# Hjinhan/Transgo

Measured on AMD Instinct MI355X. Metric: MCTS simulations/sec, higher is better.
Workload: dtype f32

## Files before the change

transgo_amd/csrc/net.hip:

```cpp
#include <cmath>
#include <cstdlib>
#include <cstring>
#include <string>
#include <vector>

#include "conv_rows.h"
#include "engine.h"

using namespace tg;

namespace tg {

struct ConvW { const float* w; const float* b; };
struct BlockW { const float* s1; const float* t1; ConvW c1; ConvW c2; const float* g1; const float* g2;
                const _Float16* h1; const _Float16* h2; };
struct AttW { ConvW qkv; const float* gamma; const float* s; const float* t;
              const _Float16* x3w = nullptr; const float* x3sc = nullptr; };
struct Layer { int kind; int ridx; AttW a; };

enum Chain { CHAIN_F32 = 0, CHAIN_DMA, CHAIN_F16, CHAIN_SPLIT };
struct NetPath {
    Chain chain = CHAIN_F32;
    bool r16 = false;
    bool att_x3 = false;
// ... 209 lines not shown
                if (m >= 0 && m < M) xreg[i] = *reinterpret_cast<const f32x4*>(in + (size_t)m * CIN + cc + c4 * 4);
            }
        }
    };
    auto store_x = [&](int cc) {
#pragma unroll
        for (int i = 0; i < XL; ++i) {
            const int idx = tid + i * 256;
            if (idx < NROW * C4) {
                const int r = idx / C4, c4 = idx % C4;
                f32x4 v = xreg[i];
                if (PRO) {
                    const int m = m0 - HALO + r;
                    if (m >= 0 && m < M) {
                        const f32x4 sc = *reinterpret_cast<const f32x4*>(ps + cc + c4 * 4);
                        const f32x4 sh = *reinterpret_cast<const f32x4*>(pt + cc + c4 * 4);
#pragma unroll
                        for (int e = 0; e < 4; ++e) { float u = v[e] * sc[e] + sh[e]; v[e] = u > 0.f ? u : 0.f; }
                    }
                }
                *reinterpret_cast<f32x4*>(&xs[r * RS + c4 * 4]) = v;
            }
        }
    };
    load_x(0);
    load_w(0, 0);
    for (int cc = 0; cc < CIN; cc += CC) {
        for (int tap = 0; tap < NTAP; ++tap) {
            if (!WALL || tap == 0) {
                __syncthreads();
                if (tap == 0) store_x(cc);
                store_w();
                __syncthreads();
                if (!WALL && tap < NTAP - 1) load_w(cc, tap + 1);
                else if (cc + CC < CIN) { load_w(cc + CC, 0); load_x(cc + CC); }
            }
            const int toff = NTAP == 9 ? (tap / 3 - 1) * S + (tap % 3 - 1) : 0;
#pragma unroll
            for (int sub = 0; sub < CC / 16; ++sub) {
                f32x4 b[NPT];
#pragma unroll
                for (int t = 0; t < NPT; ++t) {
                    const int r = (wave * NPT + t) * 16 + j + HALO + toff;
                    b[t] = *reinterpret_cast<const f32x4*>(&xs[r * RS + sub * 16 + kq * 4]);
                    if (!((vmask[t] >> tap) & 1)) b[t] = f32x4{0.f, 0.f, 0.f, 0.f};
                }
#pragma unroll
                for (int ct = 0; ct < CT; ++ct) {
                    const f32x4 a = *reinterpret_cast<const f32x4*>(&ws[((WALL ? tap * COUT : 0) + ct * 16 + j) * RS + sub * 16 + kq * 4]);
#pragma unroll
                    for (int s = 0; s < 4; ++s)
#pragma unroll
                        for (int t = 0; t < NPT; ++t)
                            acc[ct][t] = __builtin_amdgcn_mfma_f32_16x16x4f32(a[s], b[t][s], acc[ct][t], 0, 0, 0);
                }
            }
        }
    }
    int mrow[NPT], srow[NPT];
#pragma unroll
    for (int t = 0; t < NPT; ++t) {
        mrow[t] = m0 + (wave * NPT + t) * 16 + j;
        srow[t] = SM2 || SM1 ? conv_sg_row(mrow[t] / P, mrow[t] % P, P) : mrow[t];
    }
    conv_epilogue<COUT, CT, NPT, EPI, SM1, SM2>(acc, mrow, M, 0, kq, out, res, out2, par, srow, conv_sg_rows(M / P, P));
}

typedef __attribute__((address_space(3))) void tg_lds_void;
#define TG_VMCNT(N) asm volatile("s_waitcnt vmcnt(%0)" ::"n"(N) : "memory")
#define TG_BARRIER() do { asm volatile("" ::: "memory"); __builtin_amdgcn_s_barrier(); asm volatile("" ::: "memory"); } while (0)

using u32x4 = __attribute__((ext_vector_type(4))) unsigned int;
__device__ __forceinline__ u32x4 tg_rsrc(const void* base, unsigned bytes) {
    const unsigned long long a = (unsigned long long)base;
    return u32x4{(unsigned)a, (unsigned)(a >> 32) & 0xffffu, bytes, 0x00020000u};
}
__device__ __forceinline__ void tg_dma_global(const void* sbase , int voff_bytes, tg_lds_void* lds) {
    const unsigned la = __builtin_amdgcn_readfirstlane((unsigned)(unsigned long long)lds);
    asm volatile("s_mov_b32 m0, %0\n\ts_nop 0\n\tglobal_load_lds_dwordx4 %1, %2" ::"s"(la), "v"(voff_bytes), "s"(sbase) : "memory");
}
__device__ __forceinline__ void tg_dma_buffer(u32x4 rsrc, int voff_bytes, tg_lds_void* lds) {
    const unsigned la = __builtin_amdgcn_readfirstlane((unsigned)(unsigned long long)lds);
    asm volatile("s_mov_b32 m0, %0\n\ts_nop 0\n\tbuffer_load_dwordx4 %1, %2, 0 offen lds" ::"s"(la), "v"(voff_bytes), "s"(rsrc) : "memory");
}

__device__ __forceinline__ int swz64(int row) { return ((row >> 2) & 1) << 1; }

#ifdef TG_CONV_STAMP
__device__ unsigned long long g_conv_stamp[2 * 6 * 8];
#define TG_CSTAMP(i) do { __builtin_amdgcn_sched_barrier(0); if (cslot >= 0 && lane == 0) g_conv_stamp[cslot * 8 + (i)] = __builtin_readcyclecounter(); \
                          __builtin_amdgcn_sched_barrier(0); } while (0)
#else
#define TG_CSTAMP(i) do { } while (0)
#endif
template <int S, int F, int EPI, bool SIN = false, bool SOUT = false>
__global__ __launch_bounds__(256, (F == 128 ? 4 : 2)) void k_conv3x3_sg(const float* __restrict__ in, float* __restrict__ out,
                                                                       const float* __restrict__ res, const float* __restrict__ Ws,
                                                                       const float* __restrict__ bias, float* __restrict__ out2,
                                                                       const float* __restrict__ s2, const float* __restrict__ t2, int rows) {
    constexpr int P = S * S, CT = F / 16, CC = 16;
    constexpr int NPT = 2, TB = 64 * NPT;
    constexpr int WPW = CT / 4;
    constexpr int NSL = F / CC, D = 4;
    static_assert((F == 128 || F == 256) && NSL % 2 == 0, "tile geometry");
    __shared__ __attribute__((aligned(16))) float ws[D][F * CC];
    __shared__ __attribute__((aligned(16))) float par[3 * F];
    const int tid = threadIdx.x, lane = tid & 63;
    const int wave = __builtin_amdgcn_readfirstlane(tid >> 6);
    const int j = lane & 15, kq = lane >> 4;
#ifdef TG_CONV_STAMP
    const unsigned long long t_entry = __builtin_readcyclecounter();
    __builtin_amdgcn_sched_barrier(0);
#endif
    const int tpx = ((int)gridDim.x + 7) >> 3;
    const int bid = ((int)blockIdx.x & 7) * tpx + ((int)blockIdx.x >> 3);
    const int nrange = (rows + TB - 1) / TB;
    if (bid >= nrange * P) return;
    const int range = bid / P;
    const int p = conv_pos_of(bid - range * P, S);
    const int M = rows * P, Msm = conv_sg_rows(rows, P);
    constexpr bool ACT = EPI == 0 && SIN;
#ifdef TG_CONV_STAMP
    int cslot = -1;
    if (S == 9 && F == 128 && (EPI == 0 || SOUT) && wave == 0 && (range == 0 || range == 7)) {
        const int li = bid - range * P, I = S - 2;
        const int cls = li == 0 ? 0 : li == I * I ? 1 : li == I * I + 4 * I ? 2 : -1;
        if (cls >= 0) cslot = (EPI == 1 ? 6 : 0) + (range == 0 ? 0 : 3) + cls;
    }
    if (cslot >= 0 && lane == 0) g_conv_stamp[cslot * 8] = t_entry;
#endif
    static_assert(F <= 256, "one parameter triple per thread");
    const bool bn = out2 || ACT;
    float pbias = bias[tid & (F - 1)], ps2 = (bn ? s2 : bias)[tid & (F - 1)], pt2 = (bn ? t2 : bias)[tid & (F - 1)];
    __builtin_amdgcn_sched_barrier(0);
    TG_CSTAMP(1);

    const unsigned mask = conv_tap_mask(p, S);
    const int nt = conv_tap_count(mask), nst = NSL * nt;
    const unsigned long long taps = conv_tap_list(mask);
    const int inv = nt == 9 ? 7282 : nt == 6 ? 10923 : 16384;
    auto stage = [&](int k, int* sl, int* tap) {
        *sl = (k * inv) >> 16;
        *tap = (int)(taps >> (4 * (k - *sl * nt))) & 15;
    };

    const __amdgpu_buffer_rsrc_t rin = __builtin_amdgcn_make_buffer_rsrc(const_cast<float*>(in), 0, Msm * F * 4, 0x00020000);
    const int prow = lane >> 2, pchunk = (lane & 3) ^ swz64(lane >> 2);
    auto dma_w = [&](int k) {
        int sl, tap;
        stage(k, &sl, &tap);
        const float* src = Ws + (size_t)(sl * 9 + tap) * (F * CC);
#pragma unroll
        for (int i = 0; i < WPW; ++i) {
            const int pc = wave * WPW + i;
            tg_dma_global(src + pc * 16 * CC, (prow * CC + pchunk * 4) * 4, (tg_lds_void*)(&ws[k & (D - 1)][pc * 256]));
        }
    };
    const int aoff = j * CC + ((kq ^ swz64(j)) << 2);
    const int grp0 = (range * 4 + wave) * NPT;
    const bool active = grp0 * 16 < rows;
    const int boff = ((conv_sg_row(grp0 * 16 + j, p, P)) * CC + kq * 4) * 4;
    f32x4 acc[CT][NPT], b_cur[NPT], b_next[NPT];
    int sl_b = 0, sl_p = -1;
    f32x4 bsc, bsh;
    auto load_b = [&](f32x4* b, int k) {
        int sl, tap;
        stage(k, &sl, &tap);
        sl_b = sl;
        const int ty = (tap * 11) >> 5;
        const int soff = (sl * Msm + ((ty - 1) * S + (tap - 3 * ty - 1)) * 16) * (CC * 4);
#pragma unroll
        for (int t = 0; t < NPT; ++t)
            b[t] = __builtin_bit_cast(f32x4, __builtin_amdgcn_raw_buffer_load_b128(rin, (int)((unsigned)boff + (unsigned)soff + (unsigned)(t * (P * 16 * CC * 4))), 0, 0));
    };
    auto act_b = [&](f32x4* dst, const f32x4* b) {
        if (sl_b != sl_p) {
            sl_p = sl_b;
            bsc = *reinterpret_cast<const f32x4*>(par + F + sl_b * CC + kq * 4);
            bsh = *reinterpret_cast<const f32x4*>(par + 2 * F + sl_b * CC + kq * 4);
        }
#pragma unroll
        for (int t = 0; t < NPT; ++t)
#pragma unroll
            for (int e = 0; e < 4; ++e) dst[t][e] = bn_relu_unpacked(b[t][e], bsc[e], bsh[e]);
    };
    constexpr int NRES = EPI == 1 ? CT * NPT : 0;
#define TG_PAR_LANDED(PATH) asm volatile("; bias, s2, t2 landed: " PATH : "+v"(pbias), "+v"(ps2), "+v"(pt2))
    dma_w(0); dma_w(1);
    TG_CSTAMP(2);
    if (active) {
        load_b(b_cur, 0);
        __builtin_amdgcn_sched_barrier(0);
#pragma unroll
        for (int i = 0; i < CT * NPT; ++i) {
            const int ct = i / NPT, t = i % NPT;
            const int b = (grp0 + t) * 16 + j;
            [[maybe_unused]] const int m = b < rows ? b * P + p : M - 1;
            {
                acc[ct][t] = f32x4{0.f, 0.f, 0.f, 0.f};
                if constexpr (EPI == 1 && SIN) {
                    const __amdgpu_buffer_rsrc_t rres = __builtin_amdgcn_make_buffer_rsrc(const_cast<float*>(res), 0, Msm * F * 4, 0x00020000);
                    acc[ct][t] = __builtin_bit_cast(f32x4, __builtin_amdgcn_raw_buffer_load_b128(rres, (int)((unsigned)boff + (unsigned)(ct * Msm * (CC * 4)) + (unsigned)(t * (P * 16 * CC * 4))), 0, 0));
                } else if constexpr (EPI == 1) {
                    acc[ct][t] = *reinterpret_cast<const f32x4*>(res + (size_t)m * F + ct * 16 + kq * 4);
                }
            }
        }
        TG_VMCNT(NRES + NPT);
        TG_PAR_LANDED("wave with boards");
    } else {
        TG_VMCNT(0);
        TG_PAR_LANDED("wave without boards");
    }
#undef TG_PAR_LANDED
    if (tid < F) { par[tid] = pbias; par[F + tid] = bn ? ps2 : 0.f; par[2 * F + tid] = bn ? pt2 : 0.f; }
    asm volatile("s_waitcnt lgkmcnt(0)" ::: "memory");
    TG_BARRIER();
    TG_CSTAMP(3);
    if constexpr (ACT) {
        if (active) act_b(b_cur, b_cur);
        else {
#pragma unroll
            for (int t = 0; t < NPT; ++t) b_cur[t] = f32x4{0.f, 0.f, 0.f, 0.f};
        }
    }
    if (active) {
#pragma unroll
        for (int t = 0; t < NPT; ++t) {
            if constexpr (!ACT) asm volatile("" : "+v"(b_cur[t]));
            if constexpr (EPI == 1) {
#pragma unroll
                for (int ct = 0; ct < CT; ++ct) asm volatile("" : "+v"(acc[ct][t]));
            }
        }
    }
    dma_w(2); dma_w(3);

    auto walk_stage = [&](int k) {
        const float* wcur = ws[k & (D - 1)];
        load_b(b_next, k + 1);
        __builtin_amdgcn_sched_barrier(0);
        f32x4 a_cur = *reinterpret_cast<const f32x4*>(wcur + aoff);
#pragma unroll
        for (int ct = 0; ct < CT; ++ct) {
            f32x4 a_next = a_cur;
            if (ct + 1 < CT) a_next = *reinterpret_cast<const f32x4*>(wcur + (ct + 1) * 256 + aoff);
#pragma unroll
            for (int s4 = 0; s4 < 4; ++s4)
#pragma unroll
                for (int t = 0; t < NPT; ++t)
                    acc[ct][t] = __builtin_amdgcn_mfma_f32_16x16x4f32(a_cur[s4], b_cur[t][s4], acc[ct][t], 0, 0, 0);
            a_cur = a_next;
#ifdef TG_CONV_STAMP
            if (ct == 0 && k == 0) TG_CSTAMP(4);
#endif
        }
        if constexpr (ACT) {
            __builtin_amdgcn_sched_barrier(0);
            act_b(b_cur, b_next);
        } else {
            __builtin_amdgcn_sched_barrier(0);
#pragma unroll
            for (int t = 0; t < NPT; ++t) {
                asm volatile("" : "+v"(b_next[t]));
                b_cur[t] = b_next[t];
            }
        }
    };
#pragma unroll 1
    for (int k0 = 0; k0 < nst - 2; k0 += 2) {
#pragma unroll
        for (int h = 0; h < 2; ++h) {
            if (active) walk_stage(k0 + h);
            TG_VMCNT(0);
        }
        TG_BARRIER();
        if (k0 + 4 < nst) { dma_w(k0 + 4); dma_w(k0 + 5); }
    }
    if (!active) return;
    walk_stage(nst - 2);
    TG_VMCNT(0);
    constexpr bool SM = EPI == 0 || SOUT;
    const __amdgpu_buffer_rsrc_t rout = __builtin_amdgcn_make_buffer_rsrc(out, 0, (SM ? Msm : M) * F * 4, 0x00020000);
    const unsigned ostep = SM ? (unsigned)Msm * (CC * 4) : CC * 4;
    unsigned ooff[NPT];
#pragma unroll
    for (int t = 0; t < NPT; ++t) {
        const int b = (grp0 + t) * 16 + j;
        ooff[t] = b >= rows ? 0x80000000u : SM ? (unsigned)(conv_sg_row(b, p, P) * CC + kq * 4) * 4 : (unsigned)((b * P + p) * F + kq * 4) * 4;
    }
    auto store_tile = [&](int ct, f32x4 bv) {
#pragma unroll
        for (int t = 0; t < NPT; ++t) {
            f32x4 v = acc[ct][t] + bv;
            if constexpr (EPI == 0) {
#pragma unroll
                for (int e = 0; e < 4; ++e) v[e] = v[e] > 0.f ? v[e] : 0.f;
            }
            __builtin_amdgcn_raw_buffer_store_b128(__builtin_bit_cast(u32x4, v), rout, (int)(ooff[t] + (unsigned)ct * ostep), 0, 0);
        }
    };
    {
        const float* wcur = ws[(nst - 1) & (D - 1)];
        const float* pb = par + kq * 4;
        __builtin_amdgcn_sched_barrier(0);
        f32x4 a_cur = *reinterpret_cast<const f32x4*>(wcur + aoff);
#pragma unroll
        for (int ct = 0; ct < CT; ++ct) {
            f32x4 a_next = a_cur, bv = a_cur;
            if (ct + 1 < CT) a_next = *reinterpret_cast<const f32x4*>(wcur + (ct + 1) * 256 + aoff);
            if (ct > 0) bv = *reinterpret_cast<const f32x4*>(pb + (ct - 1) * 16);
#pragma unroll
            for (int s4 = 0; s4 < 4; ++s4) {
#pragma unroll
                for (int t = 0; t < NPT; ++t)
                    acc[ct][t] = __builtin_amdgcn_mfma_f32_16x16x4f32(a_cur[s4], b_cur[t][s4], acc[ct][t], 0, 0, 0);
                if (s4 == 0 && ct > 0) {
                    __builtin_amdgcn_sched_barrier(0);
                    store_tile(ct - 1, bv);
                    __builtin_amdgcn_sched_barrier(0);
                }
            }
            a_cur = a_next;
        }
        TG_CSTAMP(5);
        __builtin_amdgcn_sched_barrier(0);
        store_tile(CT - 1, *reinterpret_cast<const f32x4*>(pb + (CT - 1) * 16));
    }
#ifdef TG_CONV_STAMP
    TG_CSTAMP(6);
    TG_VMCNT(0);
    TG_CSTAMP(7);
#endif
}

__device__ __forceinline__ size_t h16_index(int m, int c, int M) { return (((size_t)(c >> 5) * 4 + ((c >> 3) & 3)) * M + m) * 8 + (c & 7); }

template <int N>
__device__ __forceinline__ void vmcnt_uniform(int n) {
    if (n >= N) TG_VMCNT(N);
    else if constexpr (N > 0) vmcnt_uniform<N - 1>(n);
}

__device__ __forceinline__ int x2_index(int c) { return ((c >> 4) << 5) + (c & 15); }
template <int F, int CT, int NPT, int EPI, bool R16, bool X2 = false>
__device__ __forceinline__ void conv_epilogue_h8(f32x4 (&acc)[CT][NPT], const int (&mrow)[NPT], int M, int co_base, int kq,
                                                 float* __restrict__ out32, _Float16* __restrict__ out16, const float* par, int pstride,
                                                 float wsc, float& amax) {
    static_assert(CT % 2 == 0, "tile pairs");
    static_assert(!(X2 && R16), "split precision keeps the f32 residual stream");
#pragma unroll
    for (int t = 0; t < NPT; ++t) {
        if (mrow[t] >= M) continue;
#pragma unroll
        for (int u = 0; u < CT / 2; ++u) {
            const int lc = u * 32 + kq * 8, col = co_base + lc;
            f32x4 v[2];
#pragma unroll
            for (int h = 0; h < 2; ++h) v[h] = (X2 ? acc[2 * u + h][t] * wsc : acc[2 * u + h][t]) + *reinterpret_cast<const f32x4*>(par + lc + 4 * h);
            h8 o;
            if constexpr (X2) {
                auto store_split = [&](const f32x4 (&w)[2]) {
                    h8 hi, lo;
#pragma unroll
                    for (int e = 0; e < 8; ++e) { const float x = w[e >> 2][e & 3]; hi[e] = (_Float16)x; lo[e] = (_Float16)(x - (float)hi[e]); }
#pragma unroll
                    for (int e = 0; e < 8; e += 2) amax = __builtin_fmaxf(amax, __builtin_fmaxf(__builtin_fabsf(w[e >> 2][e & 3]), __builtin_fabsf(w[e >> 2][(e & 3) + 1])));
                    const int c2 = x2_index(col);
                    *reinterpret_cast<h8*>(out16 + h16_index(mrow[t], c2, M)) = hi;
                    *reinterpret_cast<h8*>(out16 + h16_index(mrow[t], c2 + 16, M)) = lo;
                };
                if (EPI == 0 || EPI == 4) {
#pragma unroll
                    for (int h = 0; h < 2; ++h)
#pragma unroll
                        for (int e = 0; e < 4; ++e) v[h][e] = v[h][e] > 0.f ? v[h][e] : 0.f;
                }
                if (EPI == 0) { store_split(v); continue; }
                if (out32) {
#pragma unroll
                    for (int h = 0; h < 2; ++h) *reinterpret_cast<f32x4*>(out32 + (size_t)mrow[t] * F + col + 4 * h) = v[h];
                }
                if (out16) {
                    f32x4 w[2];
#pragma unroll
                    for (int h = 0; h < 2; ++h) {
                        const f32x4 sc = *reinterpret_cast<const f32x4*>(par + pstride + lc + 4 * h);
                        const f32x4 sh = *reinterpret_cast<const f32x4*>(par + 2 * pstride + lc + 4 * h);
#pragma unroll
                        for (int e = 0; e < 4; ++e) { const float y = v[h][e] * sc[e] + sh[e]; w[h][e] = y > 0.f ? y : 0.f; }
                    }
                    store_split(w);
                }
                continue;
            }
            if (EPI == 0) {
#pragma unroll
                for (int e = 0; e < 8; ++e) { const float w = v[e >> 2][e & 3]; o[e] = (_Float16)(w > 0.f ? w : 0.f); amax = __builtin_fmaxf(amax, w); }
                *reinterpret_cast<h8*>(out16 + h16_index(mrow[t], col, M)) = o;
            } else {
                if (EPI == 4) {
#pragma unroll
                    for (int h = 0; h < 2; ++h)
#pragma unroll
                        for (int e = 0; e < 4; ++e) v[h][e] = v[h][e] > 0.f ? v[h][e] : 0.f;
                }
                if (out32) {
                    if (R16) {
#pragma unroll
                        for (int e = 0; e < 8; ++e) { o[e] = (_Float16)v[e >> 2][e & 3]; amax = __builtin_fmaxf(amax, __builtin_fabsf(v[e >> 2][e & 3])); }
                        *reinterpret_cast<h8*>(reinterpret_cast<_Float16*>(out32) + h16_index(mrow[t], col, M)) = o;
                    } else {
#pragma unroll
// ... 1083 lines not shown
    __syncthreads();
    if (tid < nr) { float s2 = 0.f; for (int o = 0; o < A; ++o) s2 += logit[tid][o]; red[tid][1] = s2; }
    __syncthreads();
    for (int i = tid; i < nr * A; i += 256) {
        const int r = i / A, o = i % A;
        policy[(size_t)(row0 + r) * A + o] = logit[r][o] * (1.f / red[r][1]);
    }
}

struct ProfScope {
    Net* n; hipStream_t st; bool on;
    ProfScope(Net* net, hipStream_t s, double flops) : n(net), st(s), on(net->prof && net->ev_used + 2 <= net->ev.size()) {
        if (on) { (void)hipEventRecord(n->ev[n->ev_used], st); n->conv_flops += flops; n->conv_launches++; }
        else if (net->prof) n->conv_skipped++;
    }
    ~ProfScope() { if (on) { (void)hipEventRecord(n->ev[n->ev_used + 1], st); n->ev_used += 2; } }
};

template <int S, int F>
int forward_t(tg_ctx* ctx, Net* n, const float* obs, int rows, float* policy, float* value, float* own) {
    constexpr int P = S * S;
    constexpr bool WIDE = F == 128 || F == 256;
    hipStream_t st = ctx->stream;
    const int M = rows * P;
    const int grid = (M + 127) / 128;
    constexpr int NPT = F <= 128 ? 3 : 2;
    const int grid_f = (M + 64 * NPT - 1) / (64 * NPT);
    const int grid_h = (M + 255) / 256;
    constexpr int COS = F / 128;
    const int nblk_h2 = COS == 1 ? grid_h : (grid_h + 7) / 8 * 8 * COS;
    const double conv_flops = 2.0 * 9.0 * (double)F * (double)F * (double)M;
    constexpr int WQ = F / 4 + F / 4 + F;
    const bool big = (long long)M * F * 4 >= (1ll << 31);
    Chain chain = n->path.chain;
    if (chain == CHAIN_DMA && (long long)conv_sg_rows(rows, P) * F * 4 >= (1ll << 31)) chain = CHAIN_F32;
    if (chain == CHAIN_SPLIT && big) TG_FAIL(ctx, TG_ERR_ARG, "split-precision path: rows * P * F * 4 bytes must stay below 2 GiB per activation buffer");
    if (chain == CHAIN_F16 && (long long)M * F * 2 >= (1ll << 31)) TG_FAIL(ctx, TG_ERR_ARG, "fp16 path: rows * P * F * 2 bytes must stay below 2 GiB per activation buffer");
    const bool h16 = chain == CHAIN_F16 || chain == CHAIN_SPLIT, x2 = chain == CHAIN_SPLIT;
    const bool head16 = chain == CHAIN_F16 || (x2 && n->path.head_x2);
    auto wsc = [&](size_t conv) { return x2 ? n->wsc + conv : nullptr; };
    const size_t nl = n->layers.size(), nb = n->blocks.size();
    auto next_bn = [&](size_t j, const float** sn, const float** tn) -> bool {
        *sn = nullptr; *tn = nullptr;
        if (chain == CHAIN_F32) return false;
        if (j < nl && n->layers[j].kind == 0) { const BlockW& b = n->blocks[n->layers[j].ridx]; *sn = b.s1; *tn = b.t1; return true; }
        if (j == nl && head16) { *sn = n->s_end; *tn = n->t_end; return true; }
        return false;
    };

    float* x = n->bufA; float* y = n->bufB;
    const bool one = chain == CHAIN_DMA;
    auto conv_layer = [&](size_t j) { return j < nl && n->layers[j].kind == 0; };
    auto stem = [&](bool act, const float* sn, const float* tn, bool sout) {
        if constexpr (WIDE) {
            if (h16) {
                auto* k = x2 ? &k_conv3x3_h2<S, 64, F, 4, false, true> : n->path.r16 ? &k_conv3x3_h2<S, 64, F, 4, true> : &k_conv3x3_h2<S, 64, F, 4>;
                hipLaunchKernelGGL(k, dim3(nblk_h2), dim3(256), 0, st, n->x0h, x, act ? n->act16 : nullptr, nullptr, n->stem_h, n->stem.b,
                                   sn, tn, M, nblk_h2, wsc(2 * nb), n->range);
                return;
            }
            if (chain == CHAIN_DMA) {
                auto* k = sout ? &k_conv3x3<S, 16, F, false, 0, 9, 2, true, true> : &k_conv3x3<S, 16, F, false, 0, 9, 2, true>;
                hipLaunchKernelGGL(k, dim3(grid), dim3(256), 0, st, n->x0, x, nullptr, n->stem.w,
                                   n->stem.b, nullptr, nullptr, M, nullptr, nullptr, nullptr);
                return;
            }
        }
        hipLaunchKernelGGL((k_conv3x3<S, 16, F, false, 0>), dim3(grid), dim3(256), 0, st, n->x0, x, nullptr, n->stem.w, n->stem.b, nullptr, nullptr, M);
    };
    auto block = [&](const BlockW& b, int ridx, float* out, bool act, const float* sn, const float* tn, bool sin, bool sout) {
        if constexpr (WIDE) {
            if (h16) {
                auto* k1 = x2 ? &k_conv3x3_h2<S, 2 * F, F, 0, false, true> : &k_conv3x3_h2<S, F, F, 0>;
                auto* k2 = x2 ? &k_conv3x3_h2<S, 2 * F, F, 1, false, true> : n->path.r16 ? &k_conv3x3_h2<S, F, F, 1, true> : &k_conv3x3_h2<S, F, F, 1>;
                { ProfScope ps(n, st, conv_flops);
                  hipLaunchKernelGGL(k1, dim3(nblk_h2), dim3(256), 0, st, n->act16, nullptr, n->h16, nullptr, b.h1, b.c1.b, nullptr, nullptr,
                                     M, nblk_h2, wsc(2 * ridx), n->range); }
                { ProfScope ps(n, st, conv_flops);
                  hipLaunchKernelGGL(k2, dim3(nblk_h2), dim3(256), 0, st, n->h16, out, act ? n->act16 : nullptr, x, b.h2, b.c2.b, sn, tn,
                                     M, nblk_h2, wsc(2 * ridx + 1), n->range); }
                return;
            }
            if (chain == CHAIN_DMA) {
                const int grid_sd = ((rows + 127) / 128 * P + 7) / 8 * 8;
                auto* k1 = sin ? &k_conv3x3_sg<S, F, 0, true> : &k_conv3x3_sg<S, F, 0>;
                auto* k2 = sin ? (sout ? &k_conv3x3_sg<S, F, 1, true, true> : &k_conv3x3_sg<S, F, 1, true>)
                               : (sout ? &k_conv3x3_sg<S, F, 1, false, true> : &k_conv3x3_sg<S, F, 1>);
                { ProfScope ps(n, st, conv_flops);
                  hipLaunchKernelGGL(k1, dim3(grid_sd), dim3(256), 0, st, sin ? x : n->bufAct, n->bufH, nullptr, b.g1, b.c1.b, nullptr,
                                     sin ? b.s1 : nullptr, sin ? b.t1 : nullptr, rows); }
                { ProfScope ps(n, st, conv_flops);
                  hipLaunchKernelGGL(k2, dim3(grid_sd), dim3(256), 0, st, n->bufH, out, x, b.g2, b.c2.b, nullptr, nullptr, nullptr, rows); }
                return;
            }
        }
        { ProfScope ps(n, st, conv_flops);
          hipLaunchKernelGGL((k_conv3x3<S, F, F, true, 0, 9, NPT>), dim3(grid_f), dim3(256), 0, st, x, n->bufH, nullptr, b.c1.w, b.c1.b, b.s1, b.t1, M); }
        { ProfScope ps(n, st, conv_flops);
          hipLaunchKernelGGL((k_conv3x3<S, F, F, false, 1, 9, NPT>), dim3(grid_f), dim3(256), 0, st, n->bufH, out, x, b.c2.w, b.c2.b, nullptr, nullptr, M); }
    };
    auto attention = [&](const AttW& a, const float* xin, float* xout, const float* ps, const float* pt, bool act, const float* sn, const float* tn) -> int {
        if constexpr (S == 9 && F == 128) {
            if (x2) {
                constexpr int lds3 = (int)(sizeof(_Float16) * F / 16 * WQ * 32 + sizeof(float) * (WQ + 6 * F) + 4096);
                const int nwg = (rows + 3) / 4 < 256 ? (rows + 3) / 4 : 256;
                auto* k = ps ? &k_attention_x3<S, F, true> : &k_attention_x3<S, F, false>;
                hipLaunchKernelGGL(k, dim3(nwg), dim3(256), lds3, st, xin, xout, act ? n->act16 : nullptr, a.x3w, a.qkv.b, a.x3sc,
                                   a.gamma, a.s, a.t, ps, pt, sn, tn, rows, n->range);
                return 0;
            }
            if (chain == CHAIN_F16 && n->path.att_h) {
                constexpr int ldsh = (int)(sizeof(_Float16) * F / 32 * WQ * 32 + sizeof(float) * (WQ + 6 * F) + 4096);
                const int nwg = (rows + 3) / 4 < 256 ? (rows + 3) / 4 : 256;
                auto* k = ps ? &k_attention_h<S, F, true> : &k_attention_h<S, F, false>;
                hipLaunchKernelGGL(k, dim3(nwg), dim3(256), ldsh, st, xin, xout, act ? n->act16 : nullptr, a.x3w, a.qkv.b,
                                   a.gamma, a.s, a.t, ps, pt, sn, tn, rows, n->range);
                return 0;
            }
        }
        if (chain == CHAIN_F16) return -1;
        if (S != 19 && chain == CHAIN_F32 && !n->path.att_lds) return -1;
        auto* kq = ps ? &k_conv3x3<S, F, WQ, true, 2, 1> : &k_conv3x3<S, F, WQ, false, 2, 1>;
        hipLaunchKernelGGL(kq, dim3(grid), dim3(256), 0, st, xin, n->bufQ, nullptr, a.qkv.w, a.qkv.b, ps, pt, M, nullptr, nullptr, nullptr);
        if constexpr (S == 19) {
            if (x2) return -1;
            constexpr int ldst = att_t_lds<S, F>();
            hipLaunchKernelGGL((k_attention_t<S, F>), dim3(rows), dim3(256), ldst, st, n->bufQ, xin, xout,
                               act ? n->bufAct : nullptr, a.gamma, a.s, a.t, ps, pt, sn, tn, rows);
            return 0;
        } else {
        if constexpr (S == 9 && F == 256) {
            if (x2) {
                hipLaunchKernelGGL((k_attention_mfma<S, F, 2, true>), dim3((rows + 3) / 4), dim3(256), 0, st, n->bufQ, xin, xout,
                                   reinterpret_cast<float*>(act ? n->act16 : nullptr), a.gamma, a.s, a.t, ps, pt, sn, tn, rows, n->range);
                return 0;
            }
        }
        if constexpr (S == 9 && WIDE) {
            if (chain == CHAIN_DMA) {
                hipLaunchKernelGGL((k_attention_mfma<S, F, 2>), dim3((rows + 3) / 4), dim3(256), 0, st, n->bufQ, xin, xout,
                                   act ? n->bufAct : nullptr, a.gamma, a.s, a.t, ps, pt, sn, tn, rows);
                return 0;
            }
        }
        hipLaunchKernelGGL((k_attention<S, F>), dim3(rows), dim3(256), n->path.att_lds, st, n->bufQ, xin, xout, a.gamma, a.s, a.t, ps, pt);
        return 0;
        }
    };
    auto head_conv = [&](const float* in, float* outp, const float* Wg, const ConvW& cw, const float* ps, const float* pt) {
        const char* hg = getenv("TG_HEAD_GEMM");
        if (hg && atoi(hg) == 0) {
            auto* k = ps ? &k_conv3x3<S, F, 16, true, 0> : &k_conv3x3<S, F, 16, false, 0>;
            hipLaunchKernelGGL(k, dim3(grid), dim3(256), 0, st, in, outp, nullptr, cw.w, cw.b, ps, pt, M, nullptr, nullptr, nullptr);
            return;
        }
        constexpr int TMH = 64 * (S == 9 ? 3 : 4) - 2 * (S + 1);
        const int nt = (M + TMH - 1) / TMH, g = nt < 512 ? nt : 512;
        auto* k = ps ? &k_head_gemm<S, F, true> : &k_head_gemm<S, F, false>;
        hipLaunchKernelGGL(k, dim3(g), dim3(256), 0, st, in, outp, Wg, cw.b, ps, pt, M, nt);
    };

    if (h16) {
        int g0h = (int)(((size_t)M * 8 + 255) / 256); if (g0h > 65535) g0h = 65535;
        if (n->in_bits) hipLaunchKernelGGL((k_bits_to_rows_h<S>), dim3(g0h), dim3(256), 0, st, n->in_bits, n->in_slot, n->x0h, rows, n->C, n->in_words);
        else hipLaunchKernelGGL((k_obs_to_rows_h<S>), dim3(g0h), dim3(256), 0, st, obs, n->x0h, rows, n->C);
    } else {
        int g0 = (int)(((size_t)M * 16 + 255) / 256); if (g0 > 65535) g0 = 65535;
// ... 349 lines not shown
        TG_HIP(ctx, hipEventCreateWithFlags(&n->swapped, hipEventDisableTiming));
        TG_HIP(ctx, hipEventRecord(n->swapped, ctx->stream));
        TG_HIP(ctx, hipHostMalloc((void**)&n->pinned, sizeof(float) * n_floats, hipHostMallocDefault));
        n->active = 1;
        if (p.att_x3) {
            const int lds3 = (int)(sizeof(_Float16) * (size_t)F / 16 * Wq * 32 + sizeof(float) * (Wq + 6 * (size_t)F) + 4096);
            TG_HIP(ctx, hipFuncSetAttribute(reinterpret_cast<const void*>(&k_attention_x3<9, 128, false>), hipFuncAttributeMaxDynamicSharedMemorySize, lds3));
            TG_HIP(ctx, hipFuncSetAttribute(reinterpret_cast<const void*>(&k_attention_x3<9, 128, true>), hipFuncAttributeMaxDynamicSharedMemorySize, lds3));
        }
        if (p.att_h) {
            const int ldsh = (int)(sizeof(_Float16) * (size_t)F / 32 * Wq * 32 + sizeof(float) * (Wq + 6 * (size_t)F) + 4096);
            TG_HIP(ctx, hipFuncSetAttribute(reinterpret_cast<const void*>(&k_attention_h<9, 128, false>), hipFuncAttributeMaxDynamicSharedMemorySize, ldsh));
            TG_HIP(ctx, hipFuncSetAttribute(reinterpret_cast<const void*>(&k_attention_h<9, 128, true>), hipFuncAttributeMaxDynamicSharedMemorySize, ldsh));
        }
        if (any_att && prec == 0 && S == 19) {
            hipError_t er = hipSuccess;
            if (F == 128) er = hipFuncSetAttribute(reinterpret_cast<const void*>(&k_attention_t<19, 128>), hipFuncAttributeMaxDynamicSharedMemorySize, att_t_lds<19, 128>());
            if (F == 256) er = hipFuncSetAttribute(reinterpret_cast<const void*>(&k_attention_t<19, 256>), hipFuncAttributeMaxDynamicSharedMemorySize, att_t_lds<19, 256>());
            TG_HIP(ctx, er);
        }
        if (p.att_lds) {
            hipError_t er = hipSuccess;
#define TG_ATT_ATTR(SZ, FF) if (S == SZ && F == FF) er = hipFuncSetAttribute(reinterpret_cast<const void*>(&k_attention<SZ, FF>), hipFuncAttributeMaxDynamicSharedMemorySize, (int)p.att_lds)
            TG_ATT_ATTR(9, 32); TG_ATT_ATTR(9, 64); TG_ATT_ATTR(9, 128); TG_ATT_ATTR(9, 256);
#undef TG_ATT_ATTR
            TG_HIP(ctx, er);
        }
    }
    { int rc = adopt_pending(ctx, n, true); if (rc) return rc; }
    const int k = n->active ^ 1;
    { int rc = fill_weight_set(ctx, n, k, blob, ctx->stream); if (rc) return rc; }
    TG_HIP(ctx, hipStreamSynchronize(ctx->stream));
    n->active = k;
    bind_weights(n, k);
    return TG_OK;
}

int tg_net_load_async(tg_ctx* ctx, const char* arch_c, const float* blob, size_t n_floats) {
    if (!ctx || !blob || !arch_c) return TG_ERR_ARG;
    Net* n = ctx->eng ? ctx->eng->net : nullptr;
    if (!n || n->arch != arch_c || n->blob_floats != n_floats || n->prec != ctx->cfg.net_precision)
        return tg_net_load_arch(ctx, arch_c, blob, n_floats, 0);
    TG_HIP(ctx, hipSetDevice(ctx->cfg.device));
    { int rc = adopt_pending(ctx, n, true); if (rc) return rc; }
    memcpy(n->pinned, blob, sizeof(float) * n_floats);
    TG_HIP(ctx, hipStreamWaitEvent(n->side, n->swapped, 0));
    { int rc = fill_weight_set(ctx, n, n->active ^ 1, n->pinned, n->side); if (rc) return rc; }
    TG_HIP(ctx, hipEventRecord(n->loaded, n->side));
    n->pending = true;
    return TG_OK;
}

int tg_net_load_async_dev(tg_ctx* ctx, const char* arch_c, const float* d_blob, size_t n_floats) {
    if (!ctx || !d_blob || !arch_c) return TG_ERR_ARG;
    Net* n = ctx->eng ? ctx->eng->net : nullptr;
    TG_HIP(ctx, hipSetDevice(ctx->cfg.device));
    if (!n || n->arch != arch_c || n->blob_floats != n_floats || n->prec != ctx->cfg.net_precision) {
        std::vector<float> host(n_floats);
        TG_HIP(ctx, hipMemcpy(host.data(), d_blob, sizeof(float) * n_floats, hipMemcpyDeviceToHost));
        return tg_net_load_arch(ctx, arch_c, host.data(), n_floats, 0);
    }
    { int rc = adopt_pending(ctx, n, true); if (rc) return rc; }
    TG_HIP(ctx, hipStreamWaitEvent(n->side, n->swapped, 0));
    { int rc = fill_weight_set(ctx, n, n->active ^ 1, d_blob, n->side, true); if (rc) return rc; }
    TG_HIP(ctx, hipEventRecord(n->loaded, n->side));
    n->pending = true;
    return TG_OK;
}

int tg_net_load_poll(tg_ctx* ctx, int wait, int* pending) {
    if (!ctx || !ctx->eng || !ctx->eng->net) return TG_ERR_STATE;
    Net* n = ctx->eng->net;
    TG_HIP(ctx, hipSetDevice(ctx->cfg.device));
    int rc = adopt_pending(ctx, n, wait != 0);
    if (pending) *pending = n->pending ? 1 : 0;
    return rc;
}

#ifdef TG_CONV_STAMP
int tg_debug_conv_stamps(unsigned long long* out, int n) {
    if (n > 96) n = 96;
    return hipMemcpyFromSymbol(out, HIP_SYMBOL(g_conv_stamp), sizeof(unsigned long long) * n) == hipSuccess ? 0 : -1;
}
#endif
#ifdef TG_ATT_STAMP
int tg_debug_att_stamps(unsigned long long* out, int n) {
    if (n > 32) n = 32;
    return hipMemcpyFromSymbol(out, HIP_SYMBOL(g_att_stamp), sizeof(unsigned long long) * n) == hipSuccess ? 0 : -1;
}
#endif

void tg_net_destroy(tg_ctx* ctx) {
    if (!ctx || !ctx->eng || !ctx->eng->net) return;
    Net* n = ctx->eng->net;
    if (n->pending) (void)hipEventSynchronize(n->loaded);
    void* ptrs[] = {n->bufA, n->bufB, n->bufH, n->x0, n->hc, n->own, n->bufQ, n->hca, n->bufAct, n->act16, n->h16, n->x0h, n->range};
    for (void* p : ptrs) if (p) (void)hipFree(p);
    for (Net::WeightSet& w : n->sets) { void* q[] = {w.blob, w.wstage, w.wh, w.stem_h, w.head_h, w.wsc, w.head_g, w.head_ag, w.att_h, w.att_sc, w.head_x2, w.head_x2sc}; for (void* p : q) if (p) (void)hipFree(p); }
    if (n->side) (void)hipStreamDestroy(n->side);
    if (n->loaded) (void)hipEventDestroy(n->loaded);
    if (n->swapped) (void)hipEventDestroy(n->swapped);
    if (n->pinned) (void)hipHostFree(n->pinned);
    for (hipEvent_t ev : n->ev) (void)hipEventDestroy(ev);
    delete n;
    ctx->eng->net = nullptr;
}

int tg_net_adopt_ready(tg_ctx* ctx) {
    if (!ctx || !ctx->eng || !ctx->eng->net) return TG_OK;
    return adopt_pending(ctx, ctx->eng->net, false);
}

int tg_net_forward(tg_ctx* ctx, int rows) {
    Engine* e = ctx->eng;
    if (!e || !e->net) TG_FAIL(ctx, TG_ERR_STATE, "no network weights loaded (tg_net_load)");
    Net* n = e->net;
    n->in_bits = e->dev.obs_bits; n->in_slot = e->dev.row_slot; n->in_words = e->dev.obs_words;
    const int rc = forward_sym(ctx, n, nullptr, rows, e->dev.policy, e->dev.value, nullptr);
    n->in_bits = nullptr; n->in_slot = nullptr;
    return rc;
}

int tg_net_predict(tg_ctx* ctx, const float* obs, int n_rows, float* policy, float* value, float* own) {
    if (!ctx || !ctx->eng || !ctx->eng->net) { if (ctx) ctx->err = "no network weights loaded (tg_net_load)"; return TG_ERR_STATE; }
    TG_HIP(ctx, hipSetDevice(ctx->cfg.device));
    Net* n = ctx->eng->net;
    { int rc = adopt_pending(ctx, n, false); if (rc) return rc; }
    const size_t P = n->P, A = n->A, C = n->C;
    int done = 0;
    tg::DevBuf& din = ctx->env_f32; tg::DevBuf& dout = ctx->env_in;
    while (done < n_rows) {
        const int k = (n_rows - done) < n->rows_cap ? (n_rows - done) : n->rows_cap;
        if (din.reserve(sizeof(float) * k * C * P) || dout.reserve(sizeof(float) * k * (A + 1)))
            TG_FAIL(ctx, TG_ERR_HIP, "hipMalloc failed (predict scratch)");
        float* d_pol = (float*)dout.p; float* d_val = d_pol + (size_t)k * A;
        TG_HIP(ctx, hipMemcpyAsync(din.p, obs + (size_t)done * C * P, sizeof(float) * k * C * P, hipMemcpyHostToDevice, ctx->stream));
        int rc = forward_sym(ctx, n, (const float*)din.p, k, d_pol, d_val, own ? n->own : nullptr);
        if (rc) return rc;
        TG_HIP(ctx, hipMemcpyAsync(policy + (size_t)done * A, d_pol, sizeof(float) * k * A, hipMemcpyDeviceToHost, ctx->stream));
        TG_HIP(ctx, hipMemcpyAsync(value + done, d_val, sizeof(float) * k, hipMemcpyDeviceToHost, ctx->stream));
        if (own) TG_HIP(ctx, hipMemcpyAsync(own + (size_t)done * P, n->own, sizeof(float) * k * P, hipMemcpyDeviceToHost, ctx->stream));
        TG_HIP(ctx, hipStreamSynchronize(ctx->stream));
        done += k;
    }
    return TG_OK;
}


int tg_net_stream_layout(tg_ctx* ctx, int* one_stream, int* act_copy) {
    if (!ctx || !ctx->eng || !ctx->eng->net) return TG_ERR_STATE;
    const Net* n = ctx->eng->net;
    if (one_stream) *one_stream = n->path.chain == CHAIN_DMA;
    if (act_copy) *act_copy = n->bufAct != nullptr;
    return TG_OK;
}

int tg_net_range(tg_ctx* ctx, uint64_t* fp16_overflows, float* weight_absmax) {
    if (!ctx || !ctx->eng || !ctx->eng->net) return TG_ERR_STATE;
    Net* n = ctx->eng->net;
    TG_HIP(ctx, hipSetDevice(ctx->cfg.device));
    unsigned host[4] = {0, 0, 0, 0};
    TG_HIP(ctx, hipStreamSynchronize(ctx->stream));
    TG_HIP(ctx, hipMemcpy(host, n->range, sizeof(host), hipMemcpyDeviceToHost));
    if (fp16_overflows) *fp16_overflows = host[0];
    if (weight_absmax) { float f; memcpy(&f, &host[1 + n->active], sizeof(f)); *weight_absmax = f; }
    if (host[0])
// ... 41 lines not shown
```

transgo_amd/csrc/conv_rows.h:

```cpp
#pragma once

namespace tg {

constexpr int conv_sg_rows(int boards, int P) { return ((boards + 15) >> 4) * 16 * P; }
constexpr int conv_sg_row(int b, int p, int P) { return ((b >> 4) * P + p) * 16 + (b & 15); }

constexpr unsigned conv_tap_mask(int p, int S) {
    const int x = p % S, y = p / S;
    unsigned mk = 0;
    for (int tap = 0; tap < 9; ++tap) {
        const int yy = y + tap / 3 - 1, xx = x + tap % 3 - 1;
        if (yy >= 0 && yy < S && xx >= 0 && xx < S) mk |= 1u << tap;
    }
    return mk;
}
constexpr int conv_tap_count(unsigned mask) {
    int n = 0;
    for (int tap = 0; tap < 9; ++tap) n += (mask >> tap) & 1;
    return n;
}
constexpr unsigned long long conv_tap_list(unsigned mask) {
    unsigned long long l = 0;
    int k = 0;
    for (int tap = 0; tap < 9; ++tap)
        if ((mask >> tap) & 1) { l |= (unsigned long long)tap << (4 * k); ++k; }
    return l;
}

constexpr int conv_pos_of(int idx, int S) {
    const int I = S - 2;
    if (idx < I * I) return (1 + idx / I) * S + 1 + idx % I;
    const int e = idx - I * I;
    if (e < 4 * I) {
        const int side = e / I, k = 1 + e % I;
        return side == 0 ? k : side == 1 ? (S - 1) * S + k : side == 2 ? k * S : k * S + S - 1;
    }
    const int c = e - 4 * I;
    return (c >> 1) * (S - 1) * S + (c & 1) * (S - 1);
}

}
```

Baseline: 559,800.

## DMA conv epilogue parameters straight to LDS and peel the first stage pair

Bias, scale and shift are now copied straight from global memory into LDS with global_load_lds_dword, instead of being loaded into registers and written to LDS by each thread. This drops the register round trip and the lgkmcnt wait before the first barrier. The first two walk stages are also peeled into the prologue so MFMA work starts right after the first barrier, overlapping the next weight DMAs. The change risks correctness: the parameter DMA no longer zeroes s2/t2 when they are unused, and only loads s2/t2 when ACT is set, even though the out2 epilogue may read them.

```diff
diff --git a/transgo_amd/csrc/net.hip b/transgo_amd/csrc/net.hip
--- a/transgo_amd/csrc/net.hip
+++ b/transgo_amd/csrc/net.hip
@@ -315,6 +315,10 @@
 __device__ __forceinline__ void tg_dma_buffer(u32x4 rsrc, int voff_bytes, tg_lds_void* lds) {
     const unsigned la = __builtin_amdgcn_readfirstlane((unsigned)(unsigned long long)lds);
     asm volatile("s_mov_b32 m0, %0\n\ts_nop 0\n\tbuffer_load_dwordx4 %1, %2, 0 offen lds" ::"s"(la), "v"(voff_bytes), "s"(rsrc) : "memory");
+}
+__device__ __forceinline__ void tg_dma_global_b32(const void* sbase , int voff_bytes, tg_lds_void* lds) {
+    const unsigned la = __builtin_amdgcn_readfirstlane((unsigned)(unsigned long long)lds);
+    asm volatile("s_mov_b32 m0, %0\n\ts_nop 0\n\tglobal_load_lds_dword %1, %2" ::"s"(la), "v"(voff_bytes), "s"(sbase) : "memory");
 }
 
 __device__ __forceinline__ int swz64(int row) { return ((row >> 2) & 1) << 1; }
@@ -362,10 +366,18 @@
     }
     if (cslot >= 0 && lane == 0) g_conv_stamp[cslot * 8] = t_entry;
 #endif
-    static_assert(F <= 256, "one parameter triple per thread");
-    const bool bn = out2 || ACT;
-    float pbias = bias[tid & (F - 1)], ps2 = (bn ? s2 : bias)[tid & (F - 1)], pt2 = (bn ? t2 : bias)[tid & (F - 1)];
-    __builtin_amdgcn_sched_barrier(0);
+    {
+        constexpr int PPA = F / 64, NPP = (ACT ? 3 : 1) * PPA;
+#pragma unroll
+        for (int q = 0; q < (NPP + 3) / 4; ++q) {
+            const int i = q * 4 + wave;
+            if (i < NPP) {
+                const int a = i / PPA;
+                const float* src = a == 0 ? bias : a == 1 ? s2 : t2;
+                tg_dma_global_b32(src, ((i - a * PPA) * 64 + lane) * 4, (tg_lds_void*)(&par[i * 64]));
+            }
+        }
+    }
     TG_CSTAMP(1);
 
     const unsigned mask = conv_tap_mask(p, S);
@@ -418,7 +430,38 @@
             for (int e = 0; e < 4; ++e) dst[t][e] = bn_relu_unpacked(b[t][e], bsc[e], bsh[e]);
     };
     constexpr int NRES = EPI == 1 ? CT * NPT : 0;
-#define TG_PAR_LANDED(PATH) asm volatile("; bias, s2, t2 landed: " PATH : "+v"(pbias), "+v"(ps2), "+v"(pt2))
+    constexpr bool PEEL = !(EPI == 1 && !SIN);
+    auto walk_stage = [&](int k) {
+        const float* wcur = ws[k & (D - 1)];
+        load_b(b_next, k + 1);
+        __builtin_amdgcn_sched_barrier(0);
+        f32x4 a_cur = *reinterpret_cast<const f32x4*>(wcur + aoff);
+#pragma unroll
+        for (int ct = 0; ct < CT; ++ct) {
+            f32x4 a_next = a_cur;
+            if (ct + 1 < CT) a_next = *reinterpret_cast<const f32x4*>(wcur + (ct + 1) * 256 + aoff);
+#pragma unroll
+            for (int s4 = 0; s4 < 4; ++s4)
+#pragma unroll
+                for (int t = 0; t < NPT; ++t)
+                    acc[ct][t] = __builtin_amdgcn_mfma_f32_16x16x4f32(a_cur[s4], b_cur[t][s4], acc[ct][t], 0, 0, 0);
+            a_cur = a_next;
+#ifdef TG_CONV_STAMP
+            if (ct == 0 && k == 0) TG_CSTAMP(4);
+#endif
+        }
+        if constexpr (ACT) {
+            __builtin_amdgcn_sched_barrier(0);
+            act_b(b_cur, b_next);
+        } else {
+            __builtin_amdgcn_sched_barrier(0);
+#pragma unroll
+            for (int t = 0; t < NPT; ++t) {
+                asm volatile("" : "+v"(b_next[t]));
+                b_cur[t] = b_next[t];
+            }
+        }
+    };
     dma_w(0); dma_w(1);
     TG_CSTAMP(2);
     if (active) {
@@ -440,68 +483,38 @@
             }
         }
         TG_VMCNT(NRES + NPT);
-        TG_PAR_LANDED("wave with boards");
+        TG_BARRIER();
+        TG_CSTAMP(3);
+        if constexpr (ACT) act_b(b_cur, b_cur);
+        if constexpr (PEEL) {
+            walk_stage(0);
+            dma_w(2); dma_w(3);
+            walk_stage(1);
+        } else {
+#pragma unroll
+            for (int t = 0; t < NPT; ++t) {
+                asm volatile("" : "+v"(b_cur[t]));
+#pragma unroll
+                for (int ct = 0; ct < CT; ++ct) asm volatile("" : "+v"(acc[ct][t]));
+            }
+            dma_w(2); dma_w(3);
+        }
     } else {
         TG_VMCNT(0);
-        TG_PAR_LANDED("wave without boards");
-    }
-#undef TG_PAR_LANDED
-    if (tid < F) { par[tid] = pbias; par[F + tid] = bn ? ps2 : 0.f; par[2 * F + tid] = bn ? pt2 : 0.f; }
-    asm volatile("s_waitcnt lgkmcnt(0)" ::: "memory");
-    TG_BARRIER();
-    TG_CSTAMP(3);
-    if constexpr (ACT) {
-        if (active) act_b(b_cur, b_cur);
-        else {
+        TG_BARRIER();
+        if constexpr (ACT) {
 #pragma unroll
             for (int t = 0; t < NPT; ++t) b_cur[t] = f32x4{0.f, 0.f, 0.f, 0.f};
         }
-    }
-    if (active) {
-#pragma unroll
-        for (int t = 0; t < NPT; ++t) {
-            if constexpr (!ACT) asm volatile("" : "+v"(b_cur[t]));
-            if constexpr (EPI == 1) {
-#pragma unroll
-                for (int ct = 0; ct < CT; ++ct) asm volatile("" : "+v"(acc[ct][t]));
-            }
-        }
-    }
-    dma_w(2); dma_w(3);
-
-    auto walk_stage = [&](int k) {
-        const float* wcur = ws[k & (D - 1)];
-        load_b(b_next, k + 1);
-        __builtin_amdgcn_sched_barrier(0);
-        f32x4 a_cur = *reinterpret_cast<const f32x4*>(wcur + aoff);
-#pragma unroll
-        for (int ct = 0; ct < CT; ++ct) {
-            f32x4 a_next = a_cur;
-            if (ct + 1 < CT) a_next = *reinterpret_cast<const f32x4*>(wcur + (ct + 1) * 256 + aoff);
-#pragma unroll
-            for (int s4 = 0; s4 < 4; ++s4)
-#pragma unroll
-                for (int t = 0; t < NPT; ++t)
-                    acc[ct][t] = __builtin_amdgcn_mfma_f32_16x16x4f32(a_cur[s4], b_cur[t][s4], acc[ct][t], 0, 0, 0);
-            a_cur = a_next;
-#ifdef TG_CONV_STAMP
-            if (ct == 0 && k == 0) TG_CSTAMP(4);
-#endif
-        }
-        if constexpr (ACT) {
-            __builtin_amdgcn_sched_barrier(0);
-            act_b(b_cur, b_next);
-        } else {
-            __builtin_amdgcn_sched_barrier(0);
-#pragma unroll
-            for (int t = 0; t < NPT; ++t) {
-                asm volatile("" : "+v"(b_next[t]));
-                b_cur[t] = b_next[t];
-            }
-        }
-    };
+        dma_w(2); dma_w(3);
+    }
+    if constexpr (PEEL) {
+        TG_VMCNT(0);
+        TG_BARRIER();
+        dma_w(4); dma_w(5);
+    }
 #pragma unroll 1
-    for (int k0 = 0; k0 < nst - 2; k0 += 2) {
+    for (int k0 = PEEL ? 2 : 0; k0 < nst - 2; k0 += 2) {
 #pragma unroll
         for (int h = 0; h < 2; ++h) {
             if (active) walk_stage(k0 + h);
```

Measured after the change: 561,100, median of 6. About the same (+0.2%).

## Reorder conv workgroup launch so tail ranges drain by tap class across XCDs

Applied to the files above, without the earlier changes.

Replaces the simple XCD-striped block-to-(range,position) mapping with a schedule in which each XCD first processes bulk ranges, then its last K ranges and the remainder ranges grouped by tap class (interior, edge, corner). Work is spread evenly across the eight XCDs in the tail. The goal is a shorter kernel tail, where cheaper edge and corner tiles finish while expensive interior tiles are still running. It also adds stamp-only drain instrumentation. The per-block index calculation gets more expensive (a loop over classes), and L2 locality per XCD may change.

```diff
diff --git a/transgo_amd/csrc/conv_rows.h b/transgo_amd/csrc/conv_rows.h
--- a/transgo_amd/csrc/conv_rows.h
+++ b/transgo_amd/csrc/conv_rows.h
@@ -39,4 +39,35 @@
     return (c >> 1) * (S - 1) * S + (c & 1) * (S - 1);
 }
 
+constexpr int conv_class_count(int c, int S) { return c == 0 ? (S - 2) * (S - 2) : c == 1 ? 4 * (S - 2) : 4; }
+constexpr int conv_class_first(int c, int S) { return c == 0 ? 0 : c == 1 ? (S - 2) * (S - 2) : (S - 2) * (S - 2) + 4 * (S - 2); }
+constexpr int conv_launch_grid(int nrange, int S) { return 8 * ((nrange >> 3) * S * S + ((nrange & 7) * S * S + 7) / 8); }
+constexpr int conv_launch_bulk(int nrange, int S, int K) { return ((nrange >> 3) - (K < (nrange >> 3) ? K : (nrange >> 3))) * S * S; }
+constexpr int conv_xcd_share(int x, int v) { return (v - x + 7) >> 3; }
+struct conv_wg { int range, p; };
+constexpr conv_wg conv_launch_wg(int x, int i, int nrange, int S, int K) {
+    const int P = S * S, q = nrange >> 3, m = nrange & 7, kd = K < q ? K : q;
+    const int bulk = (q - kd) * P;
+    if (i < bulk) {
+        const int r = i / P;
+        return {x * q + r, conv_pos_of(i - r * P, S)};
+    }
+    int d = i - bulk;
+    for (int c = 0; c < 3; ++c) {
+        const int n = conv_class_count(c, S), f = conv_class_first(c, S);
+        if (d < kd * n) {
+            const int r = d / n;
+            return {x * q + q - kd + r, conv_pos_of(f + d - r * n, S)};
+        }
+        d -= kd * n;
+        const int j0 = conv_xcd_share(x, m * f), left = conv_xcd_share(x, m * (f + n)) - j0;
+        if (d < left) {
+            const int t = x + 8 * (j0 + d) - m * f, r = t / n;
+            return {8 * q + r, conv_pos_of(f + t - r * n, S)};
+        }
+        d -= left;
+    }
+    return {-1, 0};
 }
+
+}
diff --git a/transgo_amd/csrc/net.hip b/transgo_amd/csrc/net.hip
--- a/transgo_amd/csrc/net.hip
+++ b/transgo_amd/csrc/net.hip
@@ -321,11 +321,14 @@
 
 #ifdef TG_CONV_STAMP
 __device__ unsigned long long g_conv_stamp[2 * 6 * 8];
+constexpr int TG_DRAIN_CAP = 16384, TG_DRAIN_REC = 6;
+__device__ unsigned long long g_conv_drain[2 * TG_DRAIN_CAP * TG_DRAIN_REC];
 #define TG_CSTAMP(i) do { __builtin_amdgcn_sched_barrier(0); if (cslot >= 0 && lane == 0) g_conv_stamp[cslot * 8 + (i)] = __builtin_readcyclecounter(); \
                           __builtin_amdgcn_sched_barrier(0); } while (0)
 #else
 #define TG_CSTAMP(i) do { } while (0)
 #endif
+constexpr int conv_drain_k(int S, int F) { return S == 9 && (F == 128 || F == 256) ? 4 : 1; }
 template <int S, int F, int EPI, bool SIN = false, bool SOUT = false>
 __global__ __launch_bounds__(256, (F == 128 ? 4 : 2)) void k_conv3x3_sg(const float* __restrict__ in, float* __restrict__ out,
                                                                        const float* __restrict__ res, const float* __restrict__ Ws,
@@ -336,31 +339,39 @@
     constexpr int WPW = CT / 4;
     constexpr int NSL = F / CC, D = 4;
     static_assert((F == 128 || F == 256) && NSL % 2 == 0, "tile geometry");
+    static_assert(conv_drain_k(S, F) == 1 || conv_drain_k(S, F) == 2 || conv_drain_k(S, F) == 4, "the K that tests/test_conv_launch_order.py checks");
     __shared__ __attribute__((aligned(16))) float ws[D][F * CC];
     __shared__ __attribute__((aligned(16))) float par[3 * F];
     const int tid = threadIdx.x, lane = tid & 63;
     const int wave = __builtin_amdgcn_readfirstlane(tid >> 6);
     const int j = lane & 15, kq = lane >> 4;
 #ifdef TG_CONV_STAMP
-    const unsigned long long t_entry = __builtin_readcyclecounter();
+    const unsigned long long t_entry = __builtin_readcyclecounter(), rt_entry = __builtin_amdgcn_s_memrealtime();
     __builtin_amdgcn_sched_barrier(0);
+    unsigned long long* const drec = (EPI == 0 || SOUT) && tid == 0 && (int)blockIdx.x < TG_DRAIN_CAP
+                                         ? g_conv_drain + ((size_t)(EPI == 1 ? TG_DRAIN_CAP : 0) + blockIdx.x) * TG_DRAIN_REC : nullptr;
 #endif
-    const int tpx = ((int)gridDim.x + 7) >> 3;
-    const int bid = ((int)blockIdx.x & 7) * tpx + ((int)blockIdx.x >> 3);
     const int nrange = (rows + TB - 1) / TB;
-    if (bid >= nrange * P) return;
-    const int range = bid / P;
-    const int p = conv_pos_of(bid - range * P, S);
+    const conv_wg wg = conv_launch_wg((int)blockIdx.x & 7, (int)blockIdx.x >> 3, nrange, S, conv_drain_k(S, F));
+#ifdef TG_CONV_STAMP
+    if (drec && wg.range < 0) { drec[0] = drec[1] = t_entry; drec[2] = drec[3] = rt_entry; drec[4] = ~0ull; }
+#endif
+    if (wg.range < 0) return;
+    const int range = wg.range, p = wg.p;
     const int M = rows * P, Msm = conv_sg_rows(rows, P);
     constexpr bool ACT = EPI == 0 && SIN;
 #ifdef TG_CONV_STAMP
     int cslot = -1;
     if (S == 9 && F == 128 && (EPI == 0 || SOUT) && wave == 0 && (range == 0 || range == 7)) {
-        const int li = bid - range * P, I = S - 2;
-        const int cls = li == 0 ? 0 : li == I * I ? 1 : li == I * I + 4 * I ? 2 : -1;
+        const int cls = p == conv_pos_of(conv_class_first(0, S), S) ? 0 : p == conv_pos_of(conv_class_first(1, S), S) ? 1
+                        : p == conv_pos_of(conv_class_first(2, S), S) ? 2 : -1;
         if (cls >= 0) cslot = (EPI == 1 ? 6 : 0) + (range == 0 ? 0 : 3) + cls;
     }
     if (cslot >= 0 && lane == 0) g_conv_stamp[cslot * 8] = t_entry;
+    if (drec) {
+        drec[0] = t_entry; drec[2] = rt_entry; drec[4] = (unsigned long long)range << 32 | (unsigned)p;
+        drec[5] = (unsigned long long)__builtin_amdgcn_s_getreg((3 << 11) | 20) << 32 | __builtin_amdgcn_s_getreg((31 << 11) | 4);
+    }
 #endif
     static_assert(F <= 256, "one parameter triple per thread");
     const bool bn = out2 || ACT;
@@ -562,6 +573,7 @@
     }
 #ifdef TG_CONV_STAMP
     TG_CSTAMP(6);
+    if (drec) { drec[1] = __builtin_readcyclecounter(); drec[3] = __builtin_amdgcn_s_memrealtime(); }
     TG_VMCNT(0);
     TG_CSTAMP(7);
 #endif
@@ -1811,7 +1823,7 @@
                 return;
             }
             if (chain == CHAIN_DMA) {
-                const int grid_sd = ((rows + 127) / 128 * P + 7) / 8 * 8;
+                const int grid_sd = conv_launch_grid((rows + 127) / 128, S);
                 auto* k1 = sin ? &k_conv3x3_sg<S, F, 0, true> : &k_conv3x3_sg<S, F, 0>;
                 auto* k2 = sin ? (sout ? &k_conv3x3_sg<S, F, 1, true, true> : &k_conv3x3_sg<S, F, 1, true>)
                                : (sout ? &k_conv3x3_sg<S, F, 1, false, true> : &k_conv3x3_sg<S, F, 1>);
@@ -2327,6 +2339,11 @@
     if (n > 96) n = 96;
     return hipMemcpyFromSymbol(out, HIP_SYMBOL(g_conv_stamp), sizeof(unsigned long long) * n) == hipSuccess ? 0 : -1;
 }
+int tg_debug_conv_drain(unsigned long long* out, int epi, int n) {
+    if (n > TG_DRAIN_CAP) n = TG_DRAIN_CAP;
+    return hipMemcpyFromSymbol(out, HIP_SYMBOL(g_conv_drain), sizeof(unsigned long long) * TG_DRAIN_REC * n,
+                               sizeof(unsigned long long) * TG_DRAIN_REC * TG_DRAIN_CAP * (epi ? 1 : 0)) == hipSuccess ? 0 : -1;
+}
 #endif
 #ifdef TG_ATT_STAMP
 int tg_debug_att_stamps(unsigned long long* out, int n) {
```

After: 560,100 before, 570,400 after, median of 6. 1.8% higher.
